# jorgeMFS/HYMET

Hardware: AMD Instinct MI355X
Metric: contigs/s + Mbp/s classified, CAMI-medium, 1/2/4/8 MI355X; % HBM roofline (higher is better)
Workload: dtype u64

## Files before the change

hymet_amd/_lib.py:

```python
from __future__ import annotations

import ctypes
import os

HERE = os.path.dirname(os.path.abspath(__file__))
LIB_PATH = os.path.join(HERE, "libhymet_gpu.so")

_c = ctypes
_i64, _u64, _i32, _u32, _vp = _c.c_int64, _c.c_uint64, _c.c_int, _c.c_uint32, _c.c_void_p

_SIGS = {
    "hymet_version": (_i32, []),
    "hymet_init": (_i32, [_i32, _c.POINTER(_vp)]),
    "hymet_destroy": (_i32, [_vp]),
    "hymet_last_error": (_c.c_char_p, []),
    "hymet_set_stream": (_i32, [_vp, _vp]),
    "hymet_sync": (_i32, [_vp]),
    "hymet_prof_enable": (_i32, [_vp, _i32]),
    "hymet_prof_reset": (_i32, [_vp]),
    "hymet_prof_query": (_i32, [_vp, _c.c_char_p, _c.POINTER(_c.c_double), _c.POINTER(_i64), _c.POINTER(_c.c_double)]),
    "hymet_prof_names": (_i32, [_vp, _c.c_char_p, _i64]),
    "hymet_scratch_trim": (_i32, [_vp, _c.POINTER(_i64)]),
    "hymet_scratch_cached": (_i32, [_vp, _c.POINTER(_i64)]),
    "hymet_scratch_stats": (_i32, [_vp, _vp]),
# ... 33 lines not shown
    "hymet_mm_index_info": (_i32, [_vp, _c.POINTER(_i32), _c.POINTER(_i32), _c.POINTER(_i32), _c.POINTER(_i64)]),
    "hymet_mm_index_max_occ": (_i32, [_vp, _vp, _c.c_float, _c.POINTER(_i32)]),
    "hymet_mm_index_save": (_i32, [_vp, _vp, _c.c_char_p, _i32, _c.POINTER(_i64)]),
    "hymet_mm_index_load": (_i32, [_vp, _c.c_char_p, _i64, _c.POINTER(_vp), _c.POINTER(_i64)]),
    "hymet_mm_index_export": (_i32, [_vp, _vp, _vp, _vp]),
    "hymet_mm_map": (_i32, [_vp, _vp, _vp, _vp, _vp, _vp, _vp, _vp, _i32, _c.POINTER(_vp)]),
    "hymet_mm_result_size": (_i32, [_vp, _c.POINTER(_i64)]),
    "hymet_mm_result_copy": (_i32, [_vp, _vp, _vp, _vp]),
    "hymet_mm_result_destroy": (_i32, [_vp]),
    "hymet_paf_acc_create": (_i32, [_vp, _c.POINTER(_vp)]),
    "hymet_paf_acc_reset": (_i32, [_vp]),
    "hymet_paf_acc_destroy": (_i32, [_vp]),
    "hymet_paf_acc_info": (_i32, [_vp, _c.POINTER(_i64), _c.POINTER(_vp), _c.POINTER(_vp), _c.POINTER(_vp),
                                  _c.POINTER(_vp), _c.POINTER(_vp)]),
    "hymet_paf_acc_append": (_i32, [_vp, _vp, _vp, _i64, _i64]),
    "hymet_paf_acc_copy": (_i32, [_vp, _vp, _vp, _vp, _vp]),
    "hymet_paf_acc_field": (_i32, [_vp, _vp, _i32, _vp]),
    "hymet_mm_map_acc": (_i32, [_vp, _vp, _vp, _vp, _vp, _vp, _vp, _vp, _i32, _i32, _i32, _i32, _vp]),
    "hymet_emit_paf": (_i32, [_vp, _vp, _vp, _vp, _vp, _vp, _vp, _vp, _vp, _i64, _c.POINTER(_i64), _vp]),
    "hymet_acc_ref_counts": (_i32, [_vp, _vp, _vp]),
    "hymet_acc_classify": (_i32, [_vp, _vp, _i32, _i32] + [_vp] * 15 + [_c.POINTER(_i32)]),
    "hymet_emit_tsv": (_i32, [_vp, _i32, _i32] + [_vp] * 14 + [_i64, _c.POINTER(_i64)]),
    "hymet_mm_chain_dp": (_i32, [_vp, _vp, _vp, _i64, _i32, _i32, _i32, _i32, _i32, _c.c_float, _c.c_float, _vp, _vp]),
    "hymet_lca_ref_counts": (_i32, [_vp, _vp, _i64, _vp]),
    "hymet_lca": (_i32, [_vp, _i32, _i32] + [_vp] * 17),
}

_lib = None
_oom_hook = None


def _release_torch_cache(_user):
    try:
        import torch
        torch.cuda.empty_cache()
    except Exception:
        pass


class HymetError(RuntimeError):
    pass


def load():
    global _lib
    if _lib is not None:
# ... 125 lines not shown
```

hymet_amd/csrc/mm_asort.hip:

```cpp
#include "mm_common.hpp"
#include "sort.hpp"

namespace hymet {
namespace mm {
namespace {

constexpr int kTile = 4096;
constexpr int kPart = 16384;
constexpr int kMaxBins = 4096;

struct Seg {
    int64_t s;
    int32_t n;
    int32_t q;
};

enum { kThread = 0, kWave, kB256, kB512, kB1K, kB2K, kB4K, kB8K, kB16K, kLarge, kClasses };

__device__ __forceinline__ int seg_class(int64_t n) {
    return n <= 8 ? kThread : n <= 64 ? kWave : n <= 256 ? kB256 : n <= 512 ? kB512 : n <= 1024 ? kB1K : n <= 2048 ? kB2K
         : n <= kTile ? kB4K : kLarge;
}
__device__ __forceinline__ int seg_class_group(int64_t n) {
    return n <= kTile ? seg_class(n) : n <= 8192 ? kB8K : n <= 16384 ? kB16K : kLarge;
// ... 172 lines not shown
        __syncthreads();
        uint32_t gex = 0, gtot = 0;
#pragma unroll
        for (int k = 0; k < 16; k++) {
            const uint32_t x = wgrp[k];
            gex += k < w ? x : 0u;
            gtot += x;
        }
        if (tid == 0) gbase = gtot ? atomicAdd(n_groups, (int32_t)gtot) : 0;
        __syncthreads();
        if (ne) {
            const int64_t slot = (int64_t)gbase + gex + __popcll(nm & ((1ull << lane) - 1));
            if (slot < cap) groups[slot] = Seg{S.s + base, (int32_t)run, S.q};
        }
        __syncthreads();
    }
    publish_counters(n_groups, 1, mail);
}

#ifndef HYMET_SCATTER_SUB
#define HYMET_SCATTER_SUB 2048
#endif
constexpr int kSub = HYMET_SCATTER_SUB;

__global__ __launch_bounds__(256) void tile_scatter_kernel(const uint64_t *__restrict__ key, const uint32_t *__restrict__ val,
                                                           const int64_t *__restrict__ tile_a0, const int32_t *__restrict__ tile_q,
                                                           const int32_t *__restrict__ tile_n, const int64_t *__restrict__ qoff,
                                                           int pb, int nbins, const uint32_t *__restrict__ H,
                                                           uint64_t *__restrict__ okey, uint32_t *__restrict__ oval) {
    extern __shared__ uint64_t smem[];
    uint64_t *sk = smem;
    uint32_t *sv = reinterpret_cast<uint32_t *>(sk + kSub);
    uint32_t *c = sv + kSub;
    uint32_t *lo = c + nbins;
    __shared__ uint32_t wsum[4];
    const int tid = threadIdx.x, lane = tid & 63, w = tid >> 6;
    const int64_t a0 = tile_a0[blockIdx.x];
    const int n = tile_n[blockIdx.x];
    const uint32_t *row = H + (int64_t)blockIdx.x * nbins;
    for (int b = tid; b < nbins; b += 256) c[b] = row[b];
    const int64_t base = qoff[tile_q[blockIdx.x]];
    const int per = (nbins + 255) / 256, b0 = min(tid * per, nbins), b1 = min(b0 + per, nbins);
    for (int r0 = 0; r0 < n; r0 += kSub) {
        const int m = min(kSub, n - r0);
        for (int b = tid; b < nbins; b += 256) lo[b] = 0;
        __syncthreads();
        uint64_t kk[kSub / 256];
        uint32_t vv[kSub / 256], rk[kSub / 256];
        int bn[kSub / 256];
#pragma unroll
        for (int j = 0; j < kSub / 256; j++) {
            const int e = min(j * 256 + tid, m - 1);
            kk[j] = key[a0 + r0 + e];
            vv[j] = val[a0 + r0 + e];
        }
#pragma unroll
        for (int j = 0; j < kSub / 256; j++) {
            const bool act = j * 256 + tid < m;
            bn[j] = (int)((kk[j] >> pb) & (uint64_t)(nbins - 1));
            rk[j] = lds_rank(lo, bn[j], act);
        }
        __syncthreads();
        {
            uint32_t sum = 0;
            for (int b = b0; b < b1; b++) sum += lo[b];
            uint32_t inc = sum;
            for (int d = 1; d < 64; d <<= 1) {
                const uint32_t o = (uint32_t)__shfl_up((int)inc, d, 64);
                if (lane >= d) inc += o;
            }
            if (lane == 63) wsum[w] = inc;
            __syncthreads();
            uint32_t ex = inc - sum;
            for (int k = 0; k < w; k++) ex += wsum[k];
            for (int b = b0; b < b1; b++) {
                const uint32_t t = lo[b];
                lo[b] = ex;
                ex += t;
            }
        }
        __syncthreads();
#pragma unroll
        for (int j = 0; j < kSub / 256; j++)
            if (j * 256 + tid < m) {
                const uint32_t slot = lo[bn[j]] + rk[j];
                sk[slot] = kk[j];
                sv[slot] = vv[j];
            }
        __syncthreads();
        for (int s = tid; s < m; s += 256) {
            const uint64_t k = sk[s];
            const int b = (int)((k >> pb) & (uint64_t)(nbins - 1));
            const int64_t pos = base + c[b] + (s - lo[b]);
            okey[pos] = k;
            oval[pos] = sv[s];
        }
        __syncthreads();
        for (int b = tid; b < nbins; b += 256) c[b] += (b + 1 < nbins ? lo[b + 1] : (uint32_t)m) - lo[b];
        __syncthreads();
    }
}

__global__ __launch_bounds__(256) void group_class_kernel(const Seg *groups, int64_t G, Seg *lists, int64_t cap, int32_t *cnt,
                                                          const uint64_t *key, const uint32_t *val, AnchorOut out,
                                                          int64_t *mail) {
    Seg sg[4];
    int cls[4];
#pragma unroll
    for (int j = 0; j < 4; j++) {
        const int64_t g = (int64_t)blockIdx.x * 1024 + j * 256 + threadIdx.x;
        sg[j] = g < G ? groups[g] : Seg{0, 0, 0};
        if (sg[j].n == 1) {
            const uint64_t k = key[sg[j].s];
            out.put(sg[j].s, k, val[sg[j].s]);
            out.head(sg[j].s, k, k, true);
        }
        cls[j] = sg[j].n > 1 ? seg_class_group(sg[j].n) : -1;
    }
    block_append<4>(sg, cls, lists, cap, cnt);
    publish_counters(cnt, kClasses, mail);
}
// ... 72 lines not shown
    }
}

__device__ __forceinline__ int lds_ix(int e) { return e + (e >> 4); }

template <int N>
__device__ __forceinline__ void reg_sort(uint64_t (&k)[N]) {
#pragma unroll
    for (int w = 2; w <= N; w <<= 1)
#pragma unroll
        for (int j = w >> 1; j > 0; j >>= 1)
#pragma unroll
            for (int i = 0; i < N; i++) {
                const int l = i ^ j;
                if (l > i) {
                    const uint64_t a = k[i], b = k[l];
                    const bool up = (i & w) == 0;
                    k[i] = up ? min(a, b) : max(a, b);
                    k[l] = up ? max(a, b) : min(a, b);
                }
            }
}

template <int BLOCK, int ITEMS>
__global__ __launch_bounds__(BLOCK) void block_seg_sort_kernel(const Seg *list, const uint64_t *key, const uint32_t *val,
                                                               int nbits, int ybits, AnchorOut out) {
    constexpr int CAP = BLOCK * ITEMS;
    __shared__ uint64_t sm[CAP + CAP / 16];
    const Seg S = list[blockIdx.x];
    const int tid = threadIdx.x;
    const uint64_t lm = (1ull << nbits) - 1, ym = (1ull << ybits) - 1;
    const uint64_t hi_bits = key[S.s] & ~lm;
    {
        uint64_t kr[ITEMS];
        uint32_t vr[ITEMS];
#pragma unroll
        for (int u = 0; u < ITEMS; u++) {
            const int e = min(u * BLOCK + tid, S.n - 1);
            kr[u] = key[S.s + e];
            vr[u] = val[S.s + e];
        }
#pragma unroll
        for (int u = 0; u < ITEMS; u++) {
            const int e = u * BLOCK + tid;
            sm[lds_ix(e)] = e < S.n ? ((kr[u] & lm) << ybits | vr[u]) : ~0ull;
        }
    }
    __syncthreads();
    uint64_t k[ITEMS];
#pragma unroll
    for (int j = 0; j < ITEMS; j++) k[j] = sm[lds_ix(tid * ITEMS + j)];
    reg_sort<ITEMS>(k);
    for (int run = ITEMS; run < CAP; run <<= 1) {
        __syncthreads();
#pragma unroll
        for (int j = 0; j < ITEMS; j++) sm[lds_ix(tid * ITEMS + j)] = k[j];
        __syncthreads();
        const int o = tid * ITEMS, base = o & ~(2 * run - 1), diag = o - base;
        const int a0 = base, b0 = base + run;
        int lo = max(0, diag - run), hi = min(diag, run);
        while (lo < hi) {
            const int mid = (lo + hi) >> 1;
            if (sm[lds_ix(a0 + mid)] <= sm[lds_ix(b0 + diag - 1 - mid)]) lo = mid + 1;
            else hi = mid;
        }
        const int ai = a0 + lo, bi = b0 + diag - lo;
        const int ae = a0 + run, be = b0 + run;
#pragma unroll
        for (int j = 0; j < ITEMS; j++) {
            const int ia = ai + j, ib = bi + ITEMS - 1 - j;
            const uint64_t va = ia < ae ? sm[lds_ix(ia)] : ~0ull, vb = ib < be ? sm[lds_ix(ib)] : ~0ull;
            k[j] = min(va, vb);
        }
#pragma unroll
        for (int d = ITEMS >> 1; d > 0; d >>= 1)
#pragma unroll
            for (int i = 0; i < ITEMS; i++)
                if ((i & d) == 0) {
                    const uint64_t x = k[i], y = k[i + d];
                    k[i] = min(x, y);
                    k[i + d] = max(x, y);
                }
    }
    __syncthreads();
#pragma unroll
    for (int j = 0; j < ITEMS; j++) sm[lds_ix(tid * ITEMS + j)] = k[j];
    __syncthreads();
    for (int e = tid; e < S.n; e += BLOCK) {
        const uint64_t w = sm[lds_ix(e)], wp = sm[lds_ix(e > 0 ? e - 1 : 0)];
        out.put(S.s + e, hi_bits | w >> ybits, (uint32_t)(w & ym));
        out.head(S.s + e, hi_bits | w >> ybits, hi_bits | wp >> ybits, e == 0);
    }
}

__global__ __launch_bounds__(256) void big_gather_kernel(const Seg *list, const int64_t *dst, int pb, const uint64_t *key,
                                                         const uint32_t *val, uint64_t *tk, uint32_t *tv) {
    const Seg S = list[blockIdx.x];
    const int64_t d = dst[blockIdx.x];
    const uint64_t pm = (1ull << pb) - 1;
    for (int e = threadIdx.x; e < S.n; e += 256) {
        tk[d + e] = (uint64_t)blockIdx.x << pb | (key[S.s + e] & pm);
        tv[d + e] = val[S.s + e];
    }
}

__global__ __launch_bounds__(256) void big_put_kernel(const Seg *list, const int64_t *dst, int pb, const uint64_t *key,
                                                      const uint64_t *tk, const uint32_t *tv, AnchorOut out) {
    const Seg S = list[blockIdx.x];
    const int64_t d = dst[blockIdx.x];
// ... 18 lines not shown
            while (b > 0 && ys[b - 1] > v) {
                ys[b] = ys[b - 1];
                b--;
            }
            ys[b] = v;
        }
        for (int a = 0; a < m; a++) out.put(S.s + e + a, hi_bits | (k & pm), ys[a]);
        for (int a = m; a <= f - e; a++) out.put(S.s + e + a, hi_bits | (k & pm), tv[d + e + a]);
    }
}

__global__ void seg_len_kernel(const Seg *list, int n, uint32_t *len) {
    const int i = blockIdx.x * blockDim.x + threadIdx.x;
    if (i < n) len[i] = (uint32_t)list[i].n;
}

int bits_of(int64_t v) {
    int b = 1;
    while ((1ll << b) <= v) b++;
    return b;
}

int sort_segments(hymet_ctx *ctx, const Seg *lists, int64_t cap, const int32_t *hc, const uint64_t *key,
                  const uint32_t *val, int nbits, int ybits, const AnchorOut &out) {
    hipStream_t st = ctx->stream;
#define HY_SEG_LAUNCH(cls, kern, block)                                                                                     \
    if (hc[cls] > 0) {                                                                                                      \
        hipLaunchKernelGGL(kern, dim3((unsigned)hc[cls]), dim3(block), 0, st, lists + cls * cap, key, val, nbits, ybits, out); \
        HY_CHECK_LAUNCH(#kern);                                                                                             \
    }
    if (hc[kThread] > 0) {
        hipLaunchKernelGGL(thread_seg_sort_kernel, dim3((unsigned)cdiv(hc[kThread], 256)), dim3(256), 0, st, lists + kThread * cap,
                           hc[kThread], key, val, out);
        HY_CHECK_LAUNCH("thread_seg_sort_kernel");
    }
    if (hc[kWave] > 0) {
        hipLaunchKernelGGL(wave_seg_sort_kernel, dim3((unsigned)hc[kWave]), dim3(64), 0, st, lists + kWave * cap, key, val, out);
        HY_CHECK_LAUNCH("wave_seg_sort_kernel");
    }
    HY_SEG_LAUNCH(kB256, (block_seg_sort_kernel<64, 4>), 64)
    HY_SEG_LAUNCH(kB512, (block_seg_sort_kernel<64, 8>), 64)
#ifndef HYMET_SORT_T1K
#define HYMET_SORT_T1K 64
#endif
#ifndef HYMET_SORT_T2K
#define HYMET_SORT_T2K 128
#endif
#ifndef HYMET_SORT_T4K
#define HYMET_SORT_T4K 256
#endif
#ifndef HYMET_SORT_T8K
#define HYMET_SORT_T8K 512
#endif
    HY_SEG_LAUNCH(kB1K, (block_seg_sort_kernel<HYMET_SORT_T1K, 1024 / HYMET_SORT_T1K>), HYMET_SORT_T1K)
    HY_SEG_LAUNCH(kB2K, (block_seg_sort_kernel<HYMET_SORT_T2K, 2048 / HYMET_SORT_T2K>), HYMET_SORT_T2K)
    HY_SEG_LAUNCH(kB4K, (block_seg_sort_kernel<HYMET_SORT_T4K, 4096 / HYMET_SORT_T4K>), HYMET_SORT_T4K)
    HY_SEG_LAUNCH(kB8K, (block_seg_sort_kernel<HYMET_SORT_T8K, 8192 / HYMET_SORT_T8K>), HYMET_SORT_T8K)
    HY_SEG_LAUNCH(kB16K, (block_seg_sort_kernel<1024, 16>), 1024)
#undef HY_SEG_LAUNCH
    return HYMET_OK;
}

}

int grouped_anchor_sort(hymet_ctx *ctx, const uint64_t *key, const uint32_t *val, int64_t n, const int64_t *d_qoff, int n_q,
                        int rb, int pb, uint64_t yhi, int64_t max_qlen, uint64_t *okey, uint32_t *oval, uint64_t *ax,
                        uint64_t *ay, uint32_t *hb, uint32_t *ax32) {
    const int cs = std::max(0, 1 + rb - 12);
    const int nbins = 1 << (1 + rb - cs);
    const int gb = pb + cs;
    const int ybits = bits_of(max_qlen);
    if (n <= 0 || n_q <= 0 || 1 + rb + pb + ybits > 63) return 1;
    hipStream_t st = ctx->stream;
    const AnchorOut out{ax, ay, rb, pb, yhi, hb, ax32};
    HY_HIP(hipMemsetAsync(hb, 0, head_bits_bytes(n), st));
    DevBuf qlists, nt;
    HY_HIP(qlists.alloc(sizeof(Seg) * kClasses * (size_t)n_q, st));
    HY_HIP(nt.alloc(4 * (size_t)(n_q + 1), st));
    hipLaunchKernelGGL(query_class_kernel, dim3((unsigned)cdiv(n_q, 256)), dim3(256), 0, st, d_qoff, n_q, qlists.as<Seg>(),
                       (int64_t)n_q, ctx->dctr + kCtrQClass, nt.as<uint32_t>(), mb_dev(ctx, kMbQClass));
    HY_CHECK_LAUNCH("query_class_kernel");
    HY_HIP(hipStreamSynchronize(st));
    int32_t hq[kClasses] = {};
    for (int c = 0; c < kClasses; c++) {
        hq[c] = (int32_t)mb_read(ctx, kMbQClass + c);
        if (hq[c] < 0 || hq[c] > n_q) return hymet::fail(HYMET_E_INTERNAL, "grouped_anchor_sort: query class count > cap");
    }
    ProfScope _ps(ctx, "mm_anchor_gsort", 52.0 * (double)n);
    int rc = sort_segments(ctx, qlists.as<Seg>(), n_q, hq, key, val, 1 + rb + pb, ybits, out);
    if (rc || hq[kLarge] == 0) return rc;
    const int nl = hq[kLarge];
    const Seg *large = qlists.as<Seg>() + kLarge * (size_t)n_q;
    DevBuf tpos;
    HY_HIP(tpos.alloc(8 * (size_t)(n_q + 1), st));
    int64_t NT = 0;
    rc = exclusive_scan_u32_i64(ctx, nt.as<uint32_t>(), tpos.as<int64_t>(), n_q, &NT);
    if (rc) return rc;
    DevBuf ta0, tq, tn, H;
    HY_HIP(ta0.alloc(8 * (size_t)NT, st));
    HY_HIP(tq.alloc(4 * (size_t)NT, st));
    HY_HIP(tn.alloc(4 * (size_t)NT, st));
    HY_HIP(H.alloc(4 * (size_t)NT * nbins, st));
    hipLaunchKernelGGL(tile_map_kernel, dim3((unsigned)cdiv(nl, 256)), dim3(256), 0, st, large, nl, tpos.as<int64_t>(),
                       ta0.as<int64_t>(), tq.as<int32_t>(), tn.as<int32_t>());
    HY_CHECK_LAUNCH("tile_map_kernel");
    hipLaunchKernelGGL(tile_hist_kernel, dim3((unsigned)NT), dim3(256), 0, st, key, ta0.as<int64_t>(), tn.as<int32_t>(), gb,
                       nbins, H.as<uint32_t>());
    HY_CHECK_LAUNCH("tile_hist_kernel");
    const int64_t gcap = std::min<int64_t>(n, NT * (int64_t)nbins);
    HY_ARG(gcap < INT32_MAX, "grouped_anchor_sort: too many groups in one batch");
    DevBuf groups;
    HY_HIP(groups.alloc(sizeof(Seg) * (size_t)(gcap + 1), st));
    hipLaunchKernelGGL(query_scan_kernel, dim3((unsigned)nl), dim3(1024), 0, st, large, tpos.as<int64_t>(), nbins,
                       H.as<uint32_t>(), groups.as<Seg>(), gcap, ctx->dctr + kCtrGroups, mb_dev(ctx, kMbGroups));
    HY_CHECK_LAUNCH("query_scan_kernel");
    HY_ARG(nbins >= 1 && nbins <= kMaxBins, "grouped_anchor_sort: bin count out of range");
    hipLaunchKernelGGL(tile_scatter_kernel, dim3((unsigned)NT), dim3(256), (size_t)kSub * 12 + (size_t)nbins * 8, st, key, val, ta0.as<int64_t>(), tq.as<int32_t>(),
                       tn.as<int32_t>(), d_qoff, gb, nbins, H.as<uint32_t>(), okey, oval);
    HY_CHECK_LAUNCH("tile_scatter_kernel");
    HY_HIP(hipStreamSynchronize(st));
    const int32_t G = (int32_t)mb_read(ctx, kMbGroups);
    if (G == 0) return HYMET_OK;
    if (G < 0 || G > gcap) return hymet::fail(HYMET_E_INTERNAL, "grouped_anchor_sort: group count > cap");
    DevBuf glists;
    HY_HIP(glists.alloc(sizeof(Seg) * kClasses * (size_t)G, st));
    hipLaunchKernelGGL(group_class_kernel, dim3((unsigned)cdiv(G, 1024)), dim3(256), 0, st, groups.as<Seg>(), (int64_t)G,
                       glists.as<Seg>(), (int64_t)G, ctx->dctr + kCtrGClass, okey, oval, out, mb_dev(ctx, kMbGClass));
    HY_CHECK_LAUNCH("group_class_kernel");
    HY_HIP(hipStreamSynchronize(st));
    int32_t hg[kClasses] = {};
    for (int c = 0; c < kClasses; c++) {
        hg[c] = (int32_t)mb_read(ctx, kMbGClass + c);
        if (hg[c] < 0 || hg[c] > G) return hymet::fail(HYMET_E_INTERNAL, "grouped_anchor_sort: group class count > cap");
    }
    rc = sort_segments(ctx, glists.as<Seg>(), (int64_t)G, hg, okey, oval, gb, ybits, out);
    if (rc) return rc;
    if (hg[kLarge] > 0) {
        const int nbig = hg[kLarge];
        const Seg *big = glists.as<Seg>() + kLarge * (size_t)G;
        DevBuf blen, bdst, tk, tk2, tv, tv2;
        HY_HIP(blen.alloc(4 * (size_t)(nbig + 1), st));
        HY_HIP(bdst.alloc(8 * (size_t)(nbig + 1), st));
        hipLaunchKernelGGL(seg_len_kernel, dim3((unsigned)cdiv(nbig, 256)), dim3(256), 0, st, big, nbig, blen.as<uint32_t>());
        HY_CHECK_LAUNCH("seg_len_kernel");
        int64_t NB = 0;
        rc = exclusive_scan_u32_i64(ctx, blen.as<uint32_t>(), bdst.as<int64_t>(), nbig, &NB);
        if (rc) return rc;
        HY_HIP(tk.alloc(8 * (size_t)NB, st));
        HY_HIP(tk2.alloc(8 * (size_t)NB, st));
        HY_HIP(tv.alloc(4 * (size_t)NB, st));
        HY_HIP(tv2.alloc(4 * (size_t)NB, st));
        hipLaunchKernelGGL(big_gather_kernel, dim3((unsigned)nbig), dim3(256), 0, st, big, bdst.as<int64_t>(), gb, okey, oval,
                           tk.as<uint64_t>(), tv.as<uint32_t>());
        HY_CHECK_LAUNCH("big_gather_kernel");
        const int end_bit = gb + bits_of(nbig);
        HY_ARG(end_bit <= 64, "grouped_anchor_sort: group rank and key bits exceed 64");
        uint64_t *kk = tk.as<uint64_t>(), *kka = tk2.as<uint64_t>();
        uint32_t *vv = tv.as<uint32_t>(), *vva = tv2.as<uint32_t>();
        rc = radix_sort_pairs(ctx, kk, kka, vv, vva, NB, 0, end_bit);
        if (rc) return rc;
        hipLaunchKernelGGL(big_put_kernel, dim3((unsigned)nbig), dim3(256), 0, st, big, bdst.as<int64_t>(), gb, okey,
                           kk, vv, out);
        HY_CHECK_LAUNCH("big_put_kernel");
    }
    return HYMET_OK;
}

}
}
```

hymet_amd/csrc/mm_common.hpp:

```cpp
#pragma once
#include "common.hpp"

#include <cstring>
#include <vector>

namespace hymet {
namespace mm {

constexpr uint64_t kMax64 = ~0ull;
constexpr int kChunk = 512;

__host__ __device__ __forceinline__ uint64_t hash64m(uint64_t key, uint64_t mask) {
    key = (~key + (key << 21)) & mask;
    key = key ^ key >> 24;
    key = ((key + (key << 3)) + (key << 8)) & mask;
    key = key ^ key >> 14;
    key = ((key + (key << 2)) + (key << 4)) & mask;
    key = key ^ key >> 28;
    key = (key + (key << 31)) & mask;
    return key;
}
__host__ __device__ __forceinline__ uint64_t hash64(uint64_t key) {
    key = (~key + (key << 21));
    key = key ^ key >> 24;
// ... 80 lines not shown
    }
    __syncthreads();
    if (!last) return;
    __threadfence();
    if ((int)threadIdx.x < n) mail[threadIdx.x] = atomicExch(cnt + threadIdx.x, 0);
    if (threadIdx.x == 0) atomicExch(cnt + n, 0);
}

inline int bits_for(int64_t v) {
    int b = 0;
    while (b < 63 && (1ll << b) <= v) b++;
    return b < 1 ? 1 : b;
}
int scan_u32(hymet_ctx *ctx, const uint32_t *in, uint32_t *out, int64_t n, DevBuf &part, int64_t *mail = nullptr);
int scan_u64(hymet_ctx *ctx, const uint64_t *in, uint64_t *out, int64_t n, DevBuf &part, int64_t *mail = nullptr);
int inclusive_max_scan_i32(hymet_ctx *ctx, const int32_t *in, int32_t *out, int64_t n, DevBuf &part);

#ifndef HYMET_CHAIN_TZERO
#define HYMET_CHAIN_TZERO 0
#endif

int grouped_anchor_sort(hymet_ctx *ctx, const uint64_t *key, const uint32_t *val, int64_t n, const int64_t *d_qoff, int n_q,
                        int rb, int pb, uint64_t yhi, int64_t max_qlen, uint64_t *okey, uint32_t *oval, uint64_t *ax,
                        uint64_t *ay, uint32_t *hb, uint32_t *ax32);
inline size_t head_bits_bytes(int64_t n) { return 8 * (size_t)((n + 63) / 64 + 1); }

int sketch_sequences(hymet_ctx *ctx, const uint32_t *d_2b, const uint32_t *d_mask, const int64_t *h_starts,
                     const int64_t *h_lens, int n_seq, int w, int k, int rid_mode, DevBuf &d_x, DevBuf &d_y,
                     int64_t *n_out, DevBuf *d_seq_off);

}
}

struct hymet_mm_index {
    int w = 10, k = 15, n_seq = 0;
    int64_t n_pos = 0;
    int64_t n_buckets = 0;
    uint32_t *d_koff = nullptr;
    uint64_t *d_pos = nullptr;
    uint32_t *d_hash = nullptr;
    int64_t *d_len = nullptr;
    std::vector<int64_t> h_len;
    int device = 0;
};

struct hymet_paf_acc {
    int device = 0;
// ... 8 lines not shown
```

hymet_amd/csrc/mm_map.hip:

```cpp
#include "mm_common.hpp"
#include "sort.hpp"

#include <algorithm>
#include <type_traits>
#include <utility>

#include <chrono>
#include <cstdio>
#include <cstdlib>
#include <cstring>

struct hymet_mm_result {
    int n_q = 0;
    std::vector<int64_t> reg_off;
    std::vector<int32_t> rep_len;
    std::vector<hymet_mm_reg> regs;
};

namespace hymet {
namespace mm {

int launch_chain(hymet_ctx *ctx, const int32_t *ax, const uint64_t *ay, const int64_t *g_start, const uint8_t *g_qfirst,
                 const int32_t *order, int32_t n_work, int32_t *f, int64_t *p, int32_t *t_global, int max_dist,
                 int max_dist_inner, int bw, int max_chn_skip, int cap_rmq_size, float pen_gap, float pen_skip,
// ... 1202 lines not shown
    LAUNCH1(gather_kernel<uint64_t>, n, x.as<uint64_t>(), vv, out.ax.as<uint64_t>(), n);
    LAUNCH1(gather_kernel<uint64_t>, n, y.as<uint64_t>(), vv, out.ay.as<uint64_t>(), n);
    out.n = n;
    return HYMET_OK;
}

static int sort_anchor_keys(hymet_ctx *ctx, DevBuf &key, DevBuf &val, int64_t n, int end_bit, int rb, int pb, int yhi,
                            const int64_t *d_qoff, int n_q, int64_t max_qlen, AnchorSet &out) {
    DevBuf kb, vb;
    HY_HIP(kb.alloc(8 * (size_t)n, ctx->stream));
    HY_HIP(vb.alloc(4 * (size_t)n, ctx->stream));
    HY_HIP(out.ax.alloc(8 * (size_t)n, ctx->stream));
    HY_HIP(out.ay.alloc(8 * (size_t)n, ctx->stream));
    out.n = n;
    uint64_t *kk = key.as<uint64_t>(), *kka = kb.as<uint64_t>();
    uint32_t *vv = val.as<uint32_t>(), *vva = vb.as<uint32_t>();
    static const bool gsort = [] {
        const char *e = getenv("HYMET_ANCHOR_GSORT");
        return !(e && e[0] == '0');
    }();
    if (gsort) {
        HY_HIP(out.hb.alloc(head_bits_bytes(n), ctx->stream));
        HY_HIP(out.ax32.alloc(4 * (size_t)n, ctx->stream));
        const int rc = grouped_anchor_sort(ctx, kk, vv, n, d_qoff, n_q, rb, pb, (uint64_t)yhi, max_qlen, kka, vva,
                                           out.ax.as<uint64_t>(), out.ay.as<uint64_t>(), out.hb.as<uint32_t>(),
                                           out.ax32.as<uint32_t>());
        if (rc == HYMET_OK) {
            out.has_hb = out.has_x32 = true;
            return HYMET_OK;
        }
        if (rc != 1) return rc;
    }
    int rc = sort_pairs<uint64_t, uint32_t>(ctx, kk, kka, vv, vva, n, 0, end_bit, "radix_sort_anchors");
    if (rc) return rc;
    {
        ProfScope _ps(ctx, "mm_anchor_unpack", 28.0 * (double)n);
        LAUNCH1(anchor_unpack_kernel, n, kk, vv, n, rb, pb, (uint64_t)yhi, out.ax.as<uint64_t>(), out.ay.as<uint64_t>());
    }
    return HYMET_OK;
}

static int chain_set(hymet_ctx *ctx, const hymet_mm_opt *opt, float pen_gap, float pen_skip, int bw, AnchorSet &A,
                     int n_q, ChainSet &C, LeanJoin *lj = nullptr, bool copy = false) {
    const int64_t n = A.n;
    C.ax = A.ax.as<uint64_t>(), C.ay = A.ay.as<uint64_t>();
    if (n == 0) {
        HY_HIP(C.d_qc.alloc(8 * (size_t)(n_q + 1), ctx->stream));
        HY_HIP(C.d_qb.alloc(8 * (size_t)(n_q + 1), ctx->stream));
        HY_HIP(hipMemsetAsync(C.d_qc.p, 0, 8 * (size_t)(n_q + 1), ctx->stream));
// ... 1053 lines not shown
```

include/hymet_gpu.h:

```cpp
#ifndef HYMET_GPU_H
#define HYMET_GPU_H

#include <stdint.h>

#ifdef __cplusplus
extern "C" {
#endif

#define HYMET_OK 0
#define HYMET_E_HIP (-1)
#define HYMET_E_ARG (-2)
#define HYMET_E_CAPACITY (-3)
#define HYMET_E_INTERNAL (-4)

typedef struct hymet_ctx hymet_ctx;

int hymet_init(int device, hymet_ctx **out);
int hymet_destroy(hymet_ctx *ctx);
const char *hymet_last_error(void);
int hymet_set_stream(hymet_ctx *ctx, void *hip_stream);
int hymet_sync(hymet_ctx *ctx);
int hymet_version(void);
int hymet_prof_enable(hymet_ctx *ctx, int on);
int hymet_prof_reset(hymet_ctx *ctx);
// ... 117 lines not shown
                 hymet_mm_result **out);
int hymet_mm_result_size(const hymet_mm_result *res, int64_t *n_regs);
int hymet_mm_result_copy(const hymet_mm_result *res, int64_t *h_off, int32_t *h_rep_len,
                         hymet_mm_reg *h_regs);
int hymet_mm_result_destroy(hymet_mm_result *res);
typedef struct hymet_paf_acc hymet_paf_acc;
int hymet_paf_acc_create(hymet_ctx *ctx, hymet_paf_acc **out);
int hymet_paf_acc_reset(hymet_paf_acc *acc);
int hymet_paf_acc_destroy(hymet_paf_acc *acc);
int hymet_paf_acc_info(const hymet_paf_acc *acc, int64_t *n_lines, void **d_regs, void **d_q, void **d_part, void **d_rl,
                       void **d_t);
int hymet_paf_acc_append(hymet_ctx *ctx, hymet_paf_acc *dst, const hymet_paf_acc *src, int64_t begin, int64_t end);
int hymet_paf_acc_copy(hymet_ctx *ctx, const hymet_paf_acc *acc, int32_t *h_q, int32_t *h_part, int32_t *h_t);
int hymet_paf_acc_field(hymet_ctx *ctx, const hymet_paf_acc *acc, int field, int32_t *h_out);
int hymet_mm_map_acc(hymet_ctx *ctx, const hymet_mm_index *idx, const hymet_mm_opt *opt, const uint32_t *d_2b,
                     const uint32_t *d_mask, const int64_t *h_starts, const int64_t *h_lens, const uint32_t *d_name_hash,
                     int32_t n_q, int32_t q_base, int32_t part_id, int32_t t_base, hymet_paf_acc *acc);
int hymet_emit_paf(hymet_ctx *ctx, const hymet_paf_acc *acc, const uint8_t *d_qname, const int64_t *d_qname_off,
                   const int64_t *d_qlen, const uint8_t *d_tname, const int64_t *d_tname_off, const int64_t *d_tlen,
                   char *d_out, int64_t cap, int64_t *n_bytes, int64_t *d_line_off);
int hymet_mm_chain_dp(hymet_ctx *ctx, const uint64_t *h_x, const uint64_t *h_y, int64_t n, int max_dist,
                      int max_dist_inner, int bw, int max_chn_skip, int cap_rmq_size, float pen_gap,
                      float pen_skip, int32_t *h_f, int64_t *h_p);

int hymet_lca_ref_counts(hymet_ctx *ctx, const int32_t *d_line_t, int64_t n_lines, int32_t *d_counts);
int hymet_acc_ref_counts(hymet_ctx *ctx, const hymet_paf_acc *acc, int32_t *d_counts);
int hymet_acc_classify(hymet_ctx *ctx, const hymet_paf_acc *acc, int mode, int32_t n_q, const int64_t *d_qlen,
                       const int32_t *d_ref_counts, const int32_t *d_t_tax, const int32_t *d_tax_names,
                       const uint8_t *d_tax_in_hier, const uint8_t *d_qname_pool, const int64_t *d_qname_off,
                       const uint8_t *d_tname_pool, const int64_t *d_tname_off, int32_t *d_row_q, int32_t *d_row_part,
                       int32_t *d_row_depth, int32_t *d_row_names, double *d_row_conf, int32_t *d_row_tax,
                       int32_t *n_rows);
int hymet_emit_tsv(hymet_ctx *ctx, int mode, int32_t n_rows, const int32_t *d_row_q, const int32_t *d_row_depth,
                   const int32_t *d_row_names, const double *d_row_conf, const int32_t *d_row_tax, const uint8_t *d_qname,
                   const int64_t *d_qname_off, const uint8_t *d_label, const int64_t *d_label_off, const uint8_t *d_taxlin,
                   const int64_t *d_taxlin_off, const uint8_t *d_taxlvl, const int64_t *d_taxlvl_off, char *d_out,
                   int64_t cap, int64_t *n_bytes);
int hymet_lca(hymet_ctx *ctx, int mode, int32_t n_q, const int64_t *d_q_off, const int32_t *d_line_t,
              const int64_t *d_line_blen, const int64_t *d_line_qlen, const uint8_t *d_line_exact,
              const int32_t *d_ref_counts, const int32_t *d_t_tax, const int32_t *d_tax_names,
              const uint8_t *d_tax_in_hier, int32_t *d_scr_tid, double *d_scr_w, int32_t *d_scr_nm,
              double *d_scr_nw, int32_t *d_out_depth, int32_t *d_out_names, double *d_out_conf,
              int32_t *d_out_tax);

#ifdef __cplusplus
}
// ... 3 lines not shown
```

Measured before the change: 122,700.

## Add presortedness fast path to segment sort and wave-ordered stable tile scatter

The block segment sort now optionally detects nearly-sorted or reversed segments. It extracts up to a small number of outlier elements, sorts them with a wave bitonic network and merges them back, skipping the full merge sort when the input is almost ordered. The tile scatter gains an ordered variant that ranks with per-wave 16-bit histograms via ballot matching, which makes placement stable and wave-deterministic when LDS allows. A standalone anchor-sort entry point and optional stats counters are added for testing. The fast path adds several barrier rounds and atomics, so segments that are not nearly sorted pay extra before falling back to the full sort.

```diff
diff --git a/hymet_amd/_lib.py b/hymet_amd/_lib.py
--- a/hymet_amd/_lib.py
+++ b/hymet_amd/_lib.py
@@ -79,6 +79,7 @@
     "hymet_acc_classify": (_i32, [_vp, _vp, _i32, _i32] + [_vp] * 15 + [_c.POINTER(_i32)]),
     "hymet_emit_tsv": (_i32, [_vp, _i32, _i32] + [_vp] * 14 + [_i64, _c.POINTER(_i64)]),
     "hymet_mm_chain_dp": (_i32, [_vp, _vp, _vp, _i64, _i32, _i32, _i32, _i32, _i32, _c.c_float, _c.c_float, _vp, _vp]),
+    "hymet_mm_anchor_sort": (_i32, [_vp, _vp, _vp, _i64, _vp, _i32, _i32, _i32, _u64, _i64, _vp, _vp, _vp, _vp, _vp]),
     "hymet_lca_ref_counts": (_i32, [_vp, _vp, _i64, _vp]),
     "hymet_lca": (_i32, [_vp, _i32, _i32] + [_vp] * 17),
 }
diff --git a/hymet_amd/csrc/mm_asort.hip b/hymet_amd/csrc/mm_asort.hip
--- a/hymet_amd/csrc/mm_asort.hip
+++ b/hymet_amd/csrc/mm_asort.hip
@@ -218,7 +218,30 @@
 #define HYMET_SCATTER_SUB 2048
 #endif
 constexpr int kSub = HYMET_SCATTER_SUB;
-
+static_assert(kSub % 256 == 0 && kSub < 65536, "scatter round: whole rows of 256, 16-bit ranks");
+
+constexpr size_t scatter_lds(int nbins, bool ordered) { return (size_t)kSub * 12 + (size_t)nbins * (ordered ? 12 : 8); }
+constexpr bool scatter_ordered(int nbins) { return scatter_lds(nbins, true) <= 65536; }
+
+__device__ __forceinline__ uint32_t wave_rank_ordered(uint16_t *h, int bin, bool active, int bin_bits) {
+    const int lane = threadIdx.x & 63;
+    uint64_t peers = __ballot(active);
+    for (int i = 0; i < bin_bits; i++) {
+        const bool bit = bin >> i & 1;
+        const uint64_t m = __ballot(bit);
+        peers &= bit ? m : ~m;
+    }
+    const int leader = active ? __ffsll((unsigned long long)peers) - 1 : lane;
+    uint32_t base = 0;
+    if (active && lane == leader) {
+        base = h[bin];
+        h[bin] = (uint16_t)(base + (uint32_t)__popcll(peers));
+    }
+    base = (uint32_t)__shfl((int)base, leader, 64);
+    return base + (uint32_t)__popcll(peers & ((1ull << lane) - 1));
+}
+
+template <bool ORDERED>
 __global__ __launch_bounds__(256) void tile_scatter_kernel(const uint64_t *__restrict__ key, const uint32_t *__restrict__ val,
                                                            const int64_t *__restrict__ tile_a0, const int32_t *__restrict__ tile_q,
                                                            const int32_t *__restrict__ tile_n, const int64_t *__restrict__ qoff,
@@ -229,6 +252,7 @@
     uint32_t *sv = reinterpret_cast<uint32_t *>(sk + kSub);
     uint32_t *c = sv + kSub;
     uint32_t *lo = c + nbins;
+    uint16_t *cw = reinterpret_cast<uint16_t *>(lo);
     __shared__ uint32_t wsum[4];
     const int tid = threadIdx.x, lane = tid & 63, w = tid >> 6;
     const int64_t a0 = tile_a0[blockIdx.x];
@@ -237,29 +261,39 @@
     for (int b = tid; b < nbins; b += 256) c[b] = row[b];
     const int64_t base = qoff[tile_q[blockIdx.x]];
     const int per = (nbins + 255) / 256, b0 = min(tid * per, nbins), b1 = min(b0 + per, nbins);
+    const int bin_bits = 31 - __clz(nbins);
+    constexpr int kRows = kSub / 256;
+    const int e_first = ORDERED ? w * (kSub / 4) + lane : tid, e_step = ORDERED ? 64 : 256;
     for (int r0 = 0; r0 < n; r0 += kSub) {
         const int m = min(kSub, n - r0);
-        for (int b = tid; b < nbins; b += 256) lo[b] = 0;
-        __syncthreads();
-        uint64_t kk[kSub / 256];
-        uint32_t vv[kSub / 256], rk[kSub / 256];
-        int bn[kSub / 256];
-#pragma unroll
-        for (int j = 0; j < kSub / 256; j++) {
-            const int e = min(j * 256 + tid, m - 1);
+        if (ORDERED) {
+            for (int b = tid; b < 2 * nbins; b += 256) lo[b] = 0;
+        } else {
+            for (int b = tid; b < nbins; b += 256) lo[b] = 0;
+        }
+        __syncthreads();
+        uint64_t kk[kRows];
+        uint32_t vv[kRows], rk[kRows];
+        int bn[kRows];
+#pragma unroll
+        for (int j = 0; j < kRows; j++) {
+            const int e = min(e_first + j * e_step, m - 1);
             kk[j] = key[a0 + r0 + e];
             vv[j] = val[a0 + r0 + e];
         }
 #pragma unroll
-        for (int j = 0; j < kSub / 256; j++) {
-            const bool act = j * 256 + tid < m;
+        for (int j = 0; j < kRows; j++) {
+            const bool act = e_first + j * e_step < m;
             bn[j] = (int)((kk[j] >> pb) & (uint64_t)(nbins - 1));
-            rk[j] = lds_rank(lo, bn[j], act);
+            rk[j] = ORDERED ? wave_rank_ordered(cw + w * nbins, act ? bn[j] : 0, act, bin_bits) : lds_rank(lo, bn[j], act);
         }
         __syncthreads();
         {
             uint32_t sum = 0;
-            for (int b = b0; b < b1; b++) sum += lo[b];
+            for (int b = b0; b < b1; b++) {
+                if (ORDERED) sum += (uint32_t)cw[b] + cw[nbins + b] + cw[2 * nbins + b] + cw[3 * nbins + b];
+                else sum += lo[b];
+            }
             uint32_t inc = sum;
             for (int d = 1; d < 64; d <<= 1) {
                 const uint32_t o = (uint32_t)__shfl_up((int)inc, d, 64);
@@ -270,16 +304,25 @@
             uint32_t ex = inc - sum;
             for (int k = 0; k < w; k++) ex += wsum[k];
             for (int b = b0; b < b1; b++) {
-                const uint32_t t = lo[b];
-                lo[b] = ex;
-                ex += t;
-            }
-        }
-        __syncthreads();
-#pragma unroll
-        for (int j = 0; j < kSub / 256; j++)
-            if (j * 256 + tid < m) {
-                const uint32_t slot = lo[bn[j]] + rk[j];
+                if (ORDERED) {
+#pragma unroll
+                    for (int k = 0; k < 4; k++) {
+                        const uint32_t t = cw[k * nbins + b];
+                        cw[k * nbins + b] = (uint16_t)ex;
+                        ex += t;
+                    }
+                } else {
+                    const uint32_t t = lo[b];
+                    lo[b] = ex;
+                    ex += t;
+                }
+            }
+        }
+        __syncthreads();
+#pragma unroll
+        for (int j = 0; j < kRows; j++)
+            if (e_first + j * e_step < m) {
+                const uint32_t slot = (ORDERED ? (uint32_t)cw[w * nbins + bn[j]] : lo[bn[j]]) + rk[j];
                 sk[slot] = kk[j];
                 sv[slot] = vv[j];
             }
@@ -287,12 +330,16 @@
         for (int s = tid; s < m; s += 256) {
             const uint64_t k = sk[s];
             const int b = (int)((k >> pb) & (uint64_t)(nbins - 1));
-            const int64_t pos = base + c[b] + (s - lo[b]);
+            const int64_t pos = base + c[b] + (s - (ORDERED ? (uint32_t)cw[b] : lo[b]));
             okey[pos] = k;
             oval[pos] = sv[s];
         }
         __syncthreads();
-        for (int b = tid; b < nbins; b += 256) c[b] += (b + 1 < nbins ? lo[b + 1] : (uint32_t)m) - lo[b];
+        for (int b = tid; b < nbins; b += 256) {
+            const uint32_t cur = ORDERED ? (uint32_t)cw[b] : lo[b];
+            const uint32_t nxt = b + 1 < nbins ? (ORDERED ? (uint32_t)cw[b + 1] : lo[b + 1]) : (uint32_t)m;
+            c[b] += nxt - cur;
+        }
         __syncthreads();
     }
 }
@@ -411,15 +458,37 @@
             }
 }
 
+#ifndef HYMET_ASORT_OUTMAX
+#define HYMET_ASORT_OUTMAX 128
+#endif
+constexpr int kOutMax = HYMET_ASORT_OUTMAX;
+static_assert(kOutMax == 64 || kOutMax == 128, "the outlier sort holds one or two words per lane");
+enum { kStFastSegs = 0, kStFastAnchors, kStFullSegs, kStFullAnchors, kStats };
+
+__device__ __forceinline__ int lower_bound64(const uint64_t *o, int lo, int hi, uint64_t x) {
+    while (lo < hi) {
+        const int mid = (lo + hi) >> 1;
+        if (o[mid] < x) lo = mid + 1;
+        else hi = mid;
+    }
+    return lo;
+}
+
 template <int BLOCK, int ITEMS>
 __global__ __launch_bounds__(BLOCK) void block_seg_sort_kernel(const Seg *list, const uint64_t *key, const uint32_t *val,
-                                                               int nbits, int ybits, AnchorOut out) {
+                                                               int nbits, int ybits, AnchorOut out, int adapt,
+                                                               unsigned long long *stats) {
     constexpr int CAP = BLOCK * ITEMS;
+    static_assert(ITEMS <= 16 && BLOCK % 64 == 0, "flag words hold 16 bits per thread; whole waves");
     __shared__ uint64_t sm[CAP + CAP / 16];
+    __shared__ uint32_t fmw[BLOCK], pcnt[4], wsum[BLOCK / 64];
+    __shared__ uint64_t ol[kOutMax];
     const Seg S = list[blockIdx.x];
     const int tid = threadIdx.x;
     const uint64_t lm = (1ull << nbits) - 1, ym = (1ull << ybits) - 1;
     const uint64_t hi_bits = key[S.s] & ~lm;
+    fmw[tid] = 0;
+    if (tid < 4) pcnt[tid] = 0;
     {
         uint64_t kr[ITEMS];
         uint32_t vr[ITEMS];
@@ -437,43 +506,175 @@
     }
     __syncthreads();
     uint64_t k[ITEMS];
-#pragma unroll
-    for (int j = 0; j < ITEMS; j++) k[j] = sm[lds_ix(tid * ITEMS + j)];
-    reg_sort<ITEMS>(k);
-    for (int run = ITEMS; run < CAP; run <<= 1) {
+    bool done = false;
+    if (adapt) {
+        const int n = S.n;
+        const bool rev = sm[0] > sm[lds_ix(n - 1)];
+        auto at = [&](int e) -> uint64_t { return e < n ? sm[lds_ix(rev ? n - 1 - e : e)] : ~0ull; };
+#pragma unroll
+        for (int j = 0; j < ITEMS; j++) k[j] = at(tid * ITEMS + j);
+        constexpr uint32_t kFull = (1u << ITEMS) - 1;
+        uint32_t fl = 0;
+        int total = 0;
+        uint64_t prev = 0;
+        bool has_prev = false;
+        for (int p = 0; p < 4; p++) {
+            int pt = -1, pj = 0;
+            for (int t = tid - 1; t >= 0; t--) {
+                const uint32_t m = fmw[t] & kFull;
+                if (m != kFull) {
+                    pt = t;
+                    pj = 31 - __clz((int)(~m & kFull));
+                    break;
+                }
+            }
+            has_prev = pt >= 0;
+            prev = has_prev ? at(pt * ITEMS + pj) : 0;
+            uint32_t nf = 0;
+            uint64_t cur = prev;
+            int ct = pt, cj = pj;
+#pragma unroll
+            for (int j = 0; j < ITEMS; j++)
+                if (!(fl >> j & 1)) {
+                    if (ct >= 0 && k[j] < cur) {
+                        nf |= 1u << j;
+                        if (ct == tid) nf |= 1u << cj;
+                        else atomicOr(&fmw[ct], 0x10000u << cj);
+                    }
+                    cur = k[j];
+                    ct = tid;
+                    cj = j;
+                }
+            __syncthreads();
+            nf |= fmw[tid] >> 16;
+            fl |= nf;
+            fmw[tid] = fl;
+            if (nf) atomicAdd(&pcnt[p], (uint32_t)__popc(nf));
+            __syncthreads();
+            const int cn = (int)pcnt[p];
+            if (cn == 0) {
+                done = true;
+                break;
+            }
+            total += cn;
+            if (total > kOutMax) break;
+        }
+        if (done && total > 0) {
+            const int lane = tid & 63, w = tid >> 6;
+            const uint32_t c = (uint32_t)__popc(fl);
+            uint32_t inc = c;
+            for (int d = 1; d < 64; d <<= 1) {
+                const uint32_t o = (uint32_t)__shfl_up((int)inc, d, 64);
+                if (lane >= d) inc += o;
+            }
+            if (lane == 63) wsum[w] = inc;
+            __syncthreads();
+            uint32_t fb = inc - c;
+            for (int i = 0; i < w; i++) fb += wsum[i];
+#pragma unroll
+            for (int j = 0; j < ITEMS; j++)
+                if (fl >> j & 1) ol[fb + (uint32_t)__popc(fl & ((1u << j) - 1))] = k[j];
+            __syncthreads();
+            if (tid < 64 && total <= 64) {
+                uint64_t v = tid < total ? ol[tid] : ~0ull;
+                for (int ww = 2; ww <= 64; ww <<= 1)
+                    for (int j = ww >> 1; j > 0; j >>= 1) {
+                        const uint64_t ov = shfl_xor64(v, j);
+                        const bool up = (tid & ww) == 0, lower = (tid & j) == 0;
+                        if ((lower == up) == (ov < v)) v = ov;
+                    }
+                ol[tid] = v;
+            } else if (kOutMax > 64 && tid < 64) {
+                uint64_t v[2] = {ol[tid], tid + 64 < total ? ol[(tid + 64) % kOutMax] : ~0ull};
+                for (int ww = 2; ww <= 128; ww <<= 1)
+                    for (int j = ww >> 1; j > 0; j >>= 1) {
+                        if (j == 64) {
+                            const uint64_t a = min(v[0], v[1]), b = max(v[0], v[1]);
+                            v[0] = a;
+                            v[1] = b;
+                            continue;
+                        }
+#pragma unroll
+                        for (int r = 0; r < 2; r++) {
+                            const uint64_t ov = shfl_xor64(v[r], j);
+                            const bool up = ((tid + 64 * r) & ww) == 0, lower = (tid & j) == 0;
+                            if ((lower == up) == (ov < v[r])) v[r] = ov;
+                        }
+                    }
+                ol[tid] = v[0];
+                ol[(tid + 64) % kOutMax] = v[1];
+            }
+            __syncthreads();
+            int lcur = has_prev ? lower_bound64(ol, 0, total, prev) : 0;
+            const uint32_t kept = ~fl & kFull;
+            if (kept) {
+                uint64_t last = 0;
+#pragma unroll
+                for (int j = 0; j < ITEMS; j++)
+                    if (kept >> j & 1) last = k[j];
+                const int lend = lower_bound64(ol, lcur, total, last);
+                int r = tid * ITEMS - (int)fb;
+#pragma unroll
+                for (int j = 0; j < ITEMS; j++)
+                    if (kept >> j & 1) {
+                        const int lj = lcur == lend ? lcur : lower_bound64(ol, lcur, lend, k[j]);
+                        for (int i = lcur; i < lj; i++) sm[lds_ix(i + r)] = ol[i];
+                        sm[lds_ix(r + lj)] = k[j];
+                        lcur = lj;
+                        r++;
+                    }
+            }
+            if (tid == BLOCK - 1)
+                for (int i = lcur; i < total; i++) sm[lds_ix(i + CAP - total)] = ol[i];
+        } else if (done && rev) {
+#pragma unroll
+            for (int j = 0; j < ITEMS; j++) sm[lds_ix(tid * ITEMS + j)] = k[j];
+        }
+    } else {
+#pragma unroll
+        for (int j = 0; j < ITEMS; j++) k[j] = sm[lds_ix(tid * ITEMS + j)];
+    }
+    if (stats && tid == 0) {
+        atomicAdd(stats + (done ? kStFastSegs : kStFullSegs), 1ull);
+        atomicAdd(stats + (done ? kStFastAnchors : kStFullAnchors), (unsigned long long)S.n);
+    }
+    if (!done) {
+        reg_sort<ITEMS>(k);
+        for (int run = ITEMS; run < CAP; run <<= 1) {
+            __syncthreads();
+#pragma unroll
+            for (int j = 0; j < ITEMS; j++) sm[lds_ix(tid * ITEMS + j)] = k[j];
+            __syncthreads();
+            const int o = tid * ITEMS, base = o & ~(2 * run - 1), diag = o - base;
+            const int a0 = base, b0 = base + run;
+            int lo = max(0, diag - run), hi = min(diag, run);
+            while (lo < hi) {
+                const int mid = (lo + hi) >> 1;
+                if (sm[lds_ix(a0 + mid)] <= sm[lds_ix(b0 + diag - 1 - mid)]) lo = mid + 1;
+                else hi = mid;
+            }
+            const int ai = a0 + lo, bi = b0 + diag - lo;
+            const int ae = a0 + run, be = b0 + run;
+#pragma unroll
+            for (int j = 0; j < ITEMS; j++) {
+                const int ia = ai + j, ib = bi + ITEMS - 1 - j;
+                const uint64_t va = ia < ae ? sm[lds_ix(ia)] : ~0ull, vb = ib < be ? sm[lds_ix(ib)] : ~0ull;
+                k[j] = min(va, vb);
+            }
+#pragma unroll
+            for (int d = ITEMS >> 1; d > 0; d >>= 1)
+#pragma unroll
+                for (int i = 0; i < ITEMS; i++)
+                    if ((i & d) == 0) {
+                        const uint64_t x = k[i], y = k[i + d];
+                        k[i] = min(x, y);
+                        k[i + d] = max(x, y);
+                    }
+        }
         __syncthreads();
 #pragma unroll
         for (int j = 0; j < ITEMS; j++) sm[lds_ix(tid * ITEMS + j)] = k[j];
-        __syncthreads();
-        const int o = tid * ITEMS, base = o & ~(2 * run - 1), diag = o - base;
-        const int a0 = base, b0 = base + run;
-        int lo = max(0, diag - run), hi = min(diag, run);
-        while (lo < hi) {
-            const int mid = (lo + hi) >> 1;
-            if (sm[lds_ix(a0 + mid)] <= sm[lds_ix(b0 + diag - 1 - mid)]) lo = mid + 1;
-            else hi = mid;
-        }
-        const int ai = a0 + lo, bi = b0 + diag - lo;
-        const int ae = a0 + run, be = b0 + run;
-#pragma unroll
-        for (int j = 0; j < ITEMS; j++) {
-            const int ia = ai + j, ib = bi + ITEMS - 1 - j;
-            const uint64_t va = ia < ae ? sm[lds_ix(ia)] : ~0ull, vb = ib < be ? sm[lds_ix(ib)] : ~0ull;
-            k[j] = min(va, vb);
-        }
-#pragma unroll
-        for (int d = ITEMS >> 1; d > 0; d >>= 1)
-#pragma unroll
-            for (int i = 0; i < ITEMS; i++)
-                if ((i & d) == 0) {
-                    const uint64_t x = k[i], y = k[i + d];
-                    k[i] = min(x, y);
-                    k[i + d] = max(x, y);
-                }
-    }
-    __syncthreads();
-#pragma unroll
-    for (int j = 0; j < ITEMS; j++) sm[lds_ix(tid * ITEMS + j)] = k[j];
+    }
     __syncthreads();
     for (int e = tid; e < S.n; e += BLOCK) {
         const uint64_t w = sm[lds_ix(e)], wp = sm[lds_ix(e > 0 ? e - 1 : 0)];
@@ -538,11 +739,16 @@
 }
 
 int sort_segments(hymet_ctx *ctx, const Seg *lists, int64_t cap, const int32_t *hc, const uint64_t *key,
-                  const uint32_t *val, int nbits, int ybits, const AnchorOut &out) {
+                  const uint32_t *val, int nbits, int ybits, const AnchorOut &out, unsigned long long *stats) {
     hipStream_t st = ctx->stream;
+    static const int adapt = [] {
+        const char *e = getenv("HYMET_ASORT_ADAPT");
+        return e && e[0] == '0' ? 0 : 1;
+    }();
 #define HY_SEG_LAUNCH(cls, kern, block)                                                                                     \
     if (hc[cls] > 0) {                                                                                                      \
-        hipLaunchKernelGGL(kern, dim3((unsigned)hc[cls]), dim3(block), 0, st, lists + cls * cap, key, val, nbits, ybits, out); \
+        hipLaunchKernelGGL(kern, dim3((unsigned)hc[cls]), dim3(block), 0, st, lists + cls * cap, key, val, nbits, ybits, out, \
+                           adapt, stats);                                                                                   \
         HY_CHECK_LAUNCH(#kern);                                                                                             \
     }
     if (hc[kThread] > 0) {
@@ -581,7 +787,7 @@
 
 int grouped_anchor_sort(hymet_ctx *ctx, const uint64_t *key, const uint32_t *val, int64_t n, const int64_t *d_qoff, int n_q,
                         int rb, int pb, uint64_t yhi, int64_t max_qlen, uint64_t *okey, uint32_t *oval, uint64_t *ax,
-                        uint64_t *ay, uint32_t *hb, uint32_t *ax32) {
+                        uint64_t *ay, uint32_t *hb, uint32_t *ax32, unsigned long long *d_stats) {
     const int cs = std::max(0, 1 + rb - 12);
     const int nbins = 1 << (1 + rb - cs);
     const int gb = pb + cs;
@@ -603,7 +809,7 @@
         if (hq[c] < 0 || hq[c] > n_q) return hymet::fail(HYMET_E_INTERNAL, "grouped_anchor_sort: query class count > cap");
     }
     ProfScope _ps(ctx, "mm_anchor_gsort", 52.0 * (double)n);
-    int rc = sort_segments(ctx, qlists.as<Seg>(), n_q, hq, key, val, 1 + rb + pb, ybits, out);
+    int rc = sort_segments(ctx, qlists.as<Seg>(), n_q, hq, key, val, 1 + rb + pb, ybits, out, d_stats);
     if (rc || hq[kLarge] == 0) return rc;
     const int nl = hq[kLarge];
     const Seg *large = qlists.as<Seg>() + kLarge * (size_t)n_q;
@@ -631,8 +837,12 @@
                        H.as<uint32_t>(), groups.as<Seg>(), gcap, ctx->dctr + kCtrGroups, mb_dev(ctx, kMbGroups));
     HY_CHECK_LAUNCH("query_scan_kernel");
     HY_ARG(nbins >= 1 && nbins <= kMaxBins, "grouped_anchor_sort: bin count out of range");
-    hipLaunchKernelGGL(tile_scatter_kernel, dim3((unsigned)NT), dim3(256), (size_t)kSub * 12 + (size_t)nbins * 8, st, key, val, ta0.as<int64_t>(), tq.as<int32_t>(),
-                       tn.as<int32_t>(), d_qoff, gb, nbins, H.as<uint32_t>(), okey, oval);
+    if (scatter_ordered(nbins))
+        hipLaunchKernelGGL(tile_scatter_kernel<true>, dim3((unsigned)NT), dim3(256), scatter_lds(nbins, true), st, key, val,
+                           ta0.as<int64_t>(), tq.as<int32_t>(), tn.as<int32_t>(), d_qoff, gb, nbins, H.as<uint32_t>(), okey, oval);
+    else
+        hipLaunchKernelGGL(tile_scatter_kernel<false>, dim3((unsigned)NT), dim3(256), scatter_lds(nbins, false), st, key, val,
+                           ta0.as<int64_t>(), tq.as<int32_t>(), tn.as<int32_t>(), d_qoff, gb, nbins, H.as<uint32_t>(), okey, oval);
     HY_CHECK_LAUNCH("tile_scatter_kernel");
     HY_HIP(hipStreamSynchronize(st));
     const int32_t G = (int32_t)mb_read(ctx, kMbGroups);
@@ -649,7 +859,7 @@
         hg[c] = (int32_t)mb_read(ctx, kMbGClass + c);
         if (hg[c] < 0 || hg[c] > G) return hymet::fail(HYMET_E_INTERNAL, "grouped_anchor_sort: group class count > cap");
     }
-    rc = sort_segments(ctx, glists.as<Seg>(), (int64_t)G, hg, okey, oval, gb, ybits, out);
+    rc = sort_segments(ctx, glists.as<Seg>(), (int64_t)G, hg, okey, oval, gb, ybits, out, d_stats);
     if (rc) return rc;
     if (hg[kLarge] > 0) {
         const int nbig = hg[kLarge];
@@ -684,3 +894,48 @@
 
 }
 }
+
+extern "C" int hymet_mm_anchor_sort(hymet_ctx *ctx, const uint64_t *h_key, const uint32_t *h_val, int64_t n,
+                                    const int64_t *h_qoff, int32_t n_q, int32_t rb, int32_t pb, uint64_t yhi,
+                                    int64_t max_qlen, uint64_t *h_ax, uint64_t *h_ay, uint32_t *h_ax32, uint32_t *h_hb,
+                                    int64_t *h_stats) {
+    using hymet::mm::DevBuf;
+    HY_ARG(ctx && h_key && h_val && h_qoff && h_ax && h_ay && h_ax32 && h_hb, "hymet_mm_anchor_sort: null argument");
+    HY_ARG(n > 0 && n < INT32_MAX && n_q > 0, "hymet_mm_anchor_sort: n or n_q out of range");
+    HY_ARG(rb >= 0 && pb >= 1 && rb + pb < 63 && max_qlen >= 0, "hymet_mm_anchor_sort: key layout out of range");
+    HY_ARG(h_qoff[0] == 0 && h_qoff[n_q] == n, "hymet_mm_anchor_sort: query offsets do not span the anchors");
+    for (int32_t q = 0; q < n_q; q++) HY_ARG(h_qoff[q] <= h_qoff[q + 1], "hymet_mm_anchor_sort: query offsets not rising");
+    HY_HIP(hipSetDevice(ctx->device));
+    hipStream_t st = ctx->stream;
+    DevBuf key, val, qoff, okey, oval, ax, ay, ax32, hb, stats;
+    const size_t hb_bytes = hymet::mm::head_bits_bytes(n);
+    HY_HIP(key.alloc(8 * (size_t)n, st));
+    HY_HIP(val.alloc(4 * (size_t)n, st));
+    HY_HIP(qoff.alloc(8 * (size_t)(n_q + 1), st));
+    HY_HIP(okey.alloc(8 * (size_t)n, st));
+    HY_HIP(oval.alloc(4 * (size_t)n, st));
+    HY_HIP(ax.alloc(8 * (size_t)n, st));
+    HY_HIP(ay.alloc(8 * (size_t)n, st));
+    HY_HIP(ax32.alloc(4 * (size_t)n, st));
+    HY_HIP(hb.alloc(hb_bytes, st));
+    HY_HIP(stats.alloc(8 * hymet::mm::kStats, st));
+    HY_HIP(hipMemcpyAsync(key.p, h_key, 8 * (size_t)n, hipMemcpyHostToDevice, st));
+    HY_HIP(hipMemcpyAsync(val.p, h_val, 4 * (size_t)n, hipMemcpyHostToDevice, st));
+    HY_HIP(hipMemcpyAsync(qoff.p, h_qoff, 8 * (size_t)(n_q + 1), hipMemcpyHostToDevice, st));
+    HY_HIP(hipMemsetAsync(stats.p, 0, 8 * hymet::mm::kStats, st));
+    const int rc = hymet::mm::grouped_anchor_sort(ctx, key.as<uint64_t>(), val.as<uint32_t>(), n, qoff.as<int64_t>(), n_q, rb,
+                                                  pb, yhi, max_qlen, okey.as<uint64_t>(), oval.as<uint32_t>(),
+                                                  ax.as<uint64_t>(), ay.as<uint64_t>(), hb.as<uint32_t>(),
+                                                  ax32.as<uint32_t>(), h_stats ? stats.as<unsigned long long>() : nullptr);
+    if (rc) {
+        HY_HIP(hipStreamSynchronize(st));
+        return rc;
+    }
+    HY_HIP(hipMemcpyAsync(h_ax, ax.p, 8 * (size_t)n, hipMemcpyDeviceToHost, st));
+    HY_HIP(hipMemcpyAsync(h_ay, ay.p, 8 * (size_t)n, hipMemcpyDeviceToHost, st));
+    HY_HIP(hipMemcpyAsync(h_ax32, ax32.p, 4 * (size_t)n, hipMemcpyDeviceToHost, st));
+    HY_HIP(hipMemcpyAsync(h_hb, hb.p, 4 * (size_t)((n + 31) / 32), hipMemcpyDeviceToHost, st));
+    if (h_stats) HY_HIP(hipMemcpyAsync(h_stats, stats.p, 8 * hymet::mm::kStats, hipMemcpyDeviceToHost, st));
+    HY_HIP(hipStreamSynchronize(st));
+    return HYMET_OK;
+}
diff --git a/hymet_amd/csrc/mm_common.hpp b/hymet_amd/csrc/mm_common.hpp
--- a/hymet_amd/csrc/mm_common.hpp
+++ b/hymet_amd/csrc/mm_common.hpp
@@ -126,7 +126,7 @@
 
 int grouped_anchor_sort(hymet_ctx *ctx, const uint64_t *key, const uint32_t *val, int64_t n, const int64_t *d_qoff, int n_q,
                         int rb, int pb, uint64_t yhi, int64_t max_qlen, uint64_t *okey, uint32_t *oval, uint64_t *ax,
-                        uint64_t *ay, uint32_t *hb, uint32_t *ax32);
+                        uint64_t *ay, uint32_t *hb, uint32_t *ax32, unsigned long long *d_stats = nullptr);
 inline size_t head_bits_bytes(int64_t n) { return 8 * (size_t)((n + 63) / 64 + 1); }
 
 int sketch_sequences(hymet_ctx *ctx, const uint32_t *d_2b, const uint32_t *d_mask, const int64_t *h_starts,
diff --git a/hymet_amd/csrc/mm_map.hip b/hymet_amd/csrc/mm_map.hip
--- a/hymet_amd/csrc/mm_map.hip
+++ b/hymet_amd/csrc/mm_map.hip
@@ -1248,9 +1248,25 @@
     if (gsort) {
         HY_HIP(out.hb.alloc(head_bits_bytes(n), ctx->stream));
         HY_HIP(out.ax32.alloc(4 * (size_t)n, ctx->stream));
+        static const bool log_stats = [] {
+            const char *e = getenv("HYMET_ASORT_STATS");
+            return e && e[0] == '1';
+        }();
+        DevBuf sstat;
+        if (log_stats) {
+            HY_HIP(sstat.alloc(32, ctx->stream));
+            HY_HIP(hipMemsetAsync(sstat.p, 0, 32, ctx->stream));
+        }
         const int rc = grouped_anchor_sort(ctx, kk, vv, n, d_qoff, n_q, rb, pb, (uint64_t)yhi, max_qlen, kka, vva,
                                            out.ax.as<uint64_t>(), out.ay.as<uint64_t>(), out.hb.as<uint32_t>(),
-                                           out.ax32.as<uint32_t>());
+                                           out.ax32.as<uint32_t>(), log_stats ? sstat.as<unsigned long long>() : nullptr);
+        if (log_stats && rc == HYMET_OK) {
+            unsigned long long h[4] = {};
+            HY_HIP(hipMemcpyAsync(h, sstat.p, 32, hipMemcpyDeviceToHost, ctx->stream));
+            HY_HIP(hipStreamSynchronize(ctx->stream));
+            fprintf(stderr, "[asort] anchors %lld fast_segs %llu fast_anchors %llu full_segs %llu full_anchors %llu\n",
+                    (long long)n, h[0], h[1], h[2], h[3]);
+        }
         if (rc == HYMET_OK) {
             out.has_hb = out.has_x32 = true;
             return HYMET_OK;
diff --git a/include/hymet_gpu.h b/include/hymet_gpu.h
--- a/include/hymet_gpu.h
+++ b/include/hymet_gpu.h
@@ -163,6 +163,9 @@
 int hymet_mm_chain_dp(hymet_ctx *ctx, const uint64_t *h_x, const uint64_t *h_y, int64_t n, int max_dist,
                       int max_dist_inner, int bw, int max_chn_skip, int cap_rmq_size, float pen_gap,
                       float pen_skip, int32_t *h_f, int64_t *h_p);
+int hymet_mm_anchor_sort(hymet_ctx *ctx, const uint64_t *h_key, const uint32_t *h_val, int64_t n,
+                         const int64_t *h_qoff, int32_t n_q, int32_t rb, int32_t pb, uint64_t yhi, int64_t max_qlen,
+                         uint64_t *h_ax, uint64_t *h_ay, uint32_t *h_ax32, uint32_t *h_hb, int64_t *h_stats);
 
 int hymet_lca_ref_counts(hymet_ctx *ctx, const int32_t *d_line_t, int64_t n_lines, int32_t *d_counts);
 int hymet_acc_ref_counts(hymet_ctx *ctx, const hymet_paf_acc *acc, int32_t *d_counts);
```

After: 127,100, median of 6. +3.6%, better.
